# hitfeelee/rtm3d

Measured on AMD Instinct MI355X. Metric: images_per_sec, higher is better.
Workload: dtype fp16

## Files before the change

### rtm3d_amd/csrc/lbfgsb_wave_pub.h

```cpp
#pragma once
#include "lbfgsb.h"
#include "lbfgsb_wave.h"

#if defined(__HIPCC__)
#pragma clang fp contract(off)

namespace lbw_pub {

struct LbWaveMem {
    double ws[LB_N * LB_M], wy[LB_N * LB_M];
    double sy[LB_M * LB_M], ss[LB_M * LB_M], wt[LB_M * LB_M];
    double wn[LB_M2 * LB_M2], wn1d[LB_M2];
    double x[LB_N], z[LB_N], r[LB_N], d[LB_N], t[LB_N], g[LB_N], wv[LB_M2];
    double terms[64], fterms[16], bc[2];
    double uv[16];
#ifdef LBW_PROF
    long long prof[24];
#endif
};
#define VSY_(i, j) w->sy[((j)-1) * LB_M + (i)-1]
#define VSS_(i, j) w->ss[((j)-1) * LB_M + (i)-1]
#define VWT_(i, j) w->wt[((j)-1) * LB_M + (i)-1]
#define VWN_(i, j) w->wn[((j)-1) * LB_M2 + (i)-1]
#define VWN1_(i, j) (*((i) == (j) ? &w->wn1d[(i)-1] : &w->wn[((j)-1) * LB_M2 + (i)-1]))

struct LbWaveK { double k00, k02, k11, k12; };

__device__ static inline int lbw_opaque(int v) {
    asm volatile("" : "+v"(v));
    return v;
}

__device__ static inline int lbw_tri_col(int e) {
    int j = (int)((__fsqrt_rn(8.0f * (float)e + 1.0f) - 1.0f) * 0.5f);
    if ((j + 1) * (j + 2) / 2 <= e) ++j;
    if (j * (j + 1) / 2 > e) --j;
    return j;
}

__device__ static inline double lbw_bcast(double v, int src) {
    int lo = __double2loint(v), hi = __double2hiint(v);
    lo = __builtin_amdgcn_readlane(lo, src);
    hi = __builtin_amdgcn_readlane(hi, src);
    return __hiloint2double(hi, lo);
}

__device__ static inline double lbw_uni(double v) {
    int lo = __double2loint(v), hi = __double2hiint(v);
    lo = __builtin_amdgcn_readfirstlane(lo);
    hi = __builtin_amdgcn_readfirstlane(hi);
    return __hiloint2double(hi, lo);
}

__device__ static inline double lbw_fg(LbWaveMem* w, const LbWaveK& K, int lane) {
    const int c = lane >> 3, i = lane & 7;
    double c0, c1, c2;
    lb_corner(c, &c0, &c1, &c2);
    const double x0 = w->x[0], x1 = w->x[1], x2 = w->x[2], x3 = w->x[3], x4 = w->x[4], x5 = w->x[5], x6 = w->x[6], x7 = w->x[7];
    const double xc = c0 * x2 * x1 + c2 * x4 * x0 + x5;
    const double yc = c1 * x3 + x6;
    const double zc = (-c0) * x2 * x0 + c2 * x4 * x1 + x7;
    const double u = w->uv[2 * c], v = w->uv[2 * c + 1];
    if (i == 0) {
        const double ex = xc * K.k00 / (zc + 1e-4) + K.k02 - u;
        const double ey = yc * K.k11 / (zc + 1e-4) + K.k12 - v;
        w->fterms[2 * c] = ex * ex;
        w->fterms[2 * c + 1] = ey * ey;
    }
    const double dex = (xc * K.k00 / (zc + 1e-6) + K.k02 - u) * 2;
    const double dey = (yc * K.k11 / (zc + 1e-6) + K.k12 - v) * 2;
    double dx, dy, dz;
    switch (i) {
        case 0: dx = c2 * x4; dy = 0; dz = (-c0) * x2; break;
        case 1: dx = c0 * x2; dy = 0; dz = c2 * x4; break;
        case 2: dx = c0 * x1; dy = 0; dz = (-c0) * x0; break;
        case 3: dx = 0; dy = c1; dz = 0; break;
        case 4: dx = c2 * x0; dy = 0; dz = c2 * x1; break;
        case 5: dx = 1; dy = 0; dz = 0; break;
        case 6: dx = 0; dy = 1; dz = 0; break;
        default: dx = 0; dy = 0; dz = 1; break;
    }
    const double den = zc * zc + 1e-6;
    const double gx = K.k00 * (dx * zc - dz * xc) / den;
    const double gy = K.k11 * (dy * zc - dz * yc) / den;
    w->terms[lane] = dex * gx + dey * gy;
    WSYNC();
    if (lane < 8) {
        double s = 0.0;
        for (int k = 0; k < 8; ++k) s += w->terms[k * 8 + lane];
        w->g[lane] = s;
    }
    double f = 0.0;
    for (int k = 0; k < 16; ++k) f += w->fterms[k];
    WSYNC();
    return f;
}

__device__ static inline double lbw_dot8(const double* a, const double* b) {
    double s = 0.0;
    for (int i = 0; i < LB_N; ++i) s += a[i] * b[i];
    return s;
}

template <bool TWO>
__device__ static inline int lbw_potrf_lanes(double* a, int lda, double* b, int ldb, int n, int lane) {
    const int e = lane < (LB_M * (LB_M + 1)) / 2 ? lane : (LB_M * (LB_M + 1)) / 2 - 1;
    const int c = lbw_tri_col(e), r = e - c * (c + 1) / 2;
    const bool act = lane < (LB_M * (LB_M + 1)) / 2 && c < n;
    constexpr bool two = TWO;
    double va = act ? a[c * lda + r] : 0.0, vb = (act && two) ? b[c * ldb + r] : 0.0;
    double da = 0.0, db = 0.0;
    const int src_r = (r * (r + 1) / 2) << 2, src_c = (c * (c + 1) / 2) << 2;
    auto gather = [&](double v, int byte_idx) -> double {
        const int lo = __builtin_amdgcn_ds_bpermute(byte_idx, __double2loint(v));
        const int hi = __builtin_amdgcn_ds_bpermute(byte_idx, __double2hiint(v));
        return __hiloint2double(hi, lo);
    };
    int fail_a = LB_M, fail_b = LB_M;
#pragma unroll
    for (int k = 0; k < LB_M; ++k) {
        if (k < n) {
            const int dk = k * (k + 1) / 2 + k;
            const double pa = va - da, pb = vb - db;
            const double ajj_a = lbw_bcast(pa, dk), ajj_b = two ? lbw_bcast(pb, dk) : 1.0;
            if (!(ajj_a > 0.0) && fail_a == LB_M) fail_a = k;
            if (!(ajj_b > 0.0) && fail_b == LB_M) fail_b = k;
            const double ra = lb_rsqrt(ajj_a), rb = two ? lb_rsqrt(ajj_b) : 0.0;
            const double ua = pa * ra, ub = pb * rb;
            if (act && r == k) { va = c == k ? ra : ua; vb = c == k ? rb : ub; }
            const double ukr_a = gather(ua, src_r + (k << 2)), ukc_a = gather(ua, src_c + (k << 2));
            double ukr_b = 0.0, ukc_b = 0.0;
            if (two) { ukr_b = gather(ub, src_r + (k << 2)); ukc_b = gather(ub, src_c + (k << 2)); }
            if (act && r > k) { da += ukr_a * ukc_a; if (two) db += ukr_b * ukc_b; }
        }
    }
    if (fail_a != LB_M || fail_b != LB_M) return fail_a <= fail_b ? 1 : 2;
    if (act) { a[c * lda + r] = va; if (two) b[c * ldb + r] = vb; }
    WSYNC();
    return 0;
}

__device__ static inline int lbw_trsv_ut(const double* a, int lda, int n, double* b, double* bc, int lane) {
    (void)bc;
    const bool act = lane < n;
    const int col = (act ? lane : 0) * lda;
    double cv[LB_M2];
#pragma unroll
    for (int k = 0; k < LB_M2; ++k) cv[k] = a[col + (k < n ? k : 0)];
    const double dg = a[col + (act ? lane : 0)];
    double bj = act ? b[lane] : 0.0;
    if (__any(act && dg == 0.0)) return 1;
    double dot = 0.0;
#pragma unroll
    for (int k = 0; k < LB_M2; ++k) {
        if (k < n) {
            const double mine = (bj - dot) * dg;
            const double bk = lbw_bcast(mine, k);
            if (lane == k) bj = mine;
            if (lane > k && act) dot += cv[k] * bk;
        }
    }
    if (act) b[lane] = bj;
    WSYNC();
    return 0;
}
__device__ static inline int lbw_trsv_un(const double* a, int lda, int n, double* b, double* bc, int lane) {
    (void)bc;
    const bool act = lane < n;
    const int row = act ? lane : 0;
    constexpr int H = LB_M2 / 2;
    double rh[H], rl[H];
#pragma unroll
    for (int j = 0; j < H; ++j) rh[j] = a[((H + j) < n ? (H + j) : 0) * lda + row];
    const double dg = a[row * lda + row];
    double bk = act ? b[lane] : 0.0;
    if (__any(act && dg == 0.0)) return 1;
#pragma unroll
    for (int j = LB_M2 - 1; j >= 0; --j) {
        if (j == LB_M2 - 6) {
            asm volatile("" ::: "memory");
#pragma unroll
            for (int q = 0; q < H; ++q) rl[q] = a[(q < n ? q : 0) * lda + row];
            asm volatile("" ::: "memory");
        }
        if (j < n) {
            const double mine = bk * dg;
            const double tmp = -lbw_bcast(mine, j);
            if (lane == j) bk = mine;
            if (lane < j) bk += tmp * (j >= H ? rh[j - H] : rl[j]);
        }
    }
    if (act) b[lane] = bk;
    WSYNC();
    return 0;
}

template <bool FULL>
__device__ static inline int lbw_rhs_solve_t(const double* u, double* b, int n) {
    double bv[LB_M], acc[LB_M];
    int bad = 0;
#pragma unroll
    for (int j = 0; j < LB_M; ++j) {
        bv[j] = b[(FULL || j < n) ? j : 0];
        acc[j] = 0.0;
        if ((FULL || j < n) && u[j * LB_M2 + j] == 0.0) bad = 1;
    }
    if (bad) return 1;
#pragma unroll
    for (int J = 0; J < LB_M; ++J) {
        if (FULL || J < n) {
            asm volatile("" ::: "memory");
            double ur[LB_M];
#pragma unroll
            for (int Jp = J; Jp < LB_M; ++Jp) ur[Jp] = u[((FULL || Jp < n) ? Jp : J) * LB_M2 + J];
            const double xJ = (bv[J] - acc[J]) * ur[J];
            bv[J] = xJ;
#pragma unroll
            for (int Jp = J + 1; Jp < LB_M; ++Jp)
                if (FULL || Jp < n) acc[Jp] += ur[Jp] * xJ;
        }
    }
#pragma unroll
    for (int j = 0; j < LB_M; ++j) if (FULL || j < n) b[j] = bv[j];
    return 0;
}
__device__ static inline int lbw_rhs_solve(const double* u, double* b, int n) {
    return n == LB_M ? lbw_rhs_solve_t<true>(u, b, n) : lbw_rhs_solve_t<false>(u, b, n);
}

__device__ static inline int lbw_formk(LbWaveMem* w, int iupdat, double theta, int col, int head, int lane) {
    lane = lbw_opaque(lane);
    const int m = LB_M, n = LB_N;
    PTB(f0_);
    if (iupdat > m) {
        double v[6]; int dr[6], dc[6]; bool ok[6];
#pragma unroll
        for (int r = 0; r < 2; ++r) {
            const int e = lane + 64 * r;
            const bool in = e < (m - 1) * (m - 1);
            const int ee = in ? e : 0;
            const int c = ee / (m - 1) + 1, q = ee % (m - 1) + 1;
            const int qs = q >= c ? q : c;
            ok[3 * r + 0] = in && q >= c; v[3 * r + 0] = VWN1_(qs + 1, c + 1);         dr[3 * r + 0] = qs;     dc[3 * r + 0] = c;
            ok[3 * r + 1] = in && q >= c; v[3 * r + 1] = VWN1_(m + qs + 1, m + c + 1); dr[3 * r + 1] = m + qs; dc[3 * r + 1] = m + c;
            ok[3 * r + 2] = in;           v[3 * r + 2] = VWN1_(m + q + 1, c + 1);      dr[3 * r + 2] = m + q;  dc[3 * r + 2] = c;
        }
        WSYNC();
#pragma unroll
        for (int q = 0; q < 6; ++q) if (ok[q]) VWN1_(dr[q], dc[q]) = v[q];
        WSYNC();
    }
    PTE(f0_, 8); PTB(f1_);
    {
        int ipntr = head + col - 1;
        if (ipntr > m) ipntr -= m;
        const int jy = lane + 1;
        if (jy <= col) {
            const int jpntr = (head + jy - 2) % m + 1;
            double temp1 = 0.0;
            for (int k = 1; k <= n; ++k) temp1 += VWY_(k, ipntr) * VWY_(k, jpntr);
            VWN1_(col, jy) = temp1;
            VWN1_(m + col, m + jy) = 0.0;
            VWN1_(m + col, jy) = 0.0;
        }
        WSYNC();
        const int i = lane + 1;
        if (i <= col) {
            const int ip = (head + i - 2) % m + 1;
            double temp3 = 0.0;
            for (int k = 1; k <= n; ++k) temp3 += VWS_(k, ip) * VWY_(k, ipntr);
            VWN1_(m + i, col) = temp3;
        }
        WSYNC();
    }
    PTE(f1_, 9); PTB(f2_);
    const float rcol = 1.0f / (float)col;
    for (int e = lane; e < col * col; e += 64) {
        const int q = (int)(((float)e + 0.5f) * rcol);
        const int iy = q + 1, jy = e - q * col + 1;
        const int is = col + iy, is1 = m + iy, js = col + jy, js1 = m + jy;
        if (jy <= iy) {
            double v = VWN1_(iy, jy) / theta;
            if (jy == iy) v = v + VSY_(iy, iy);
            VWN_(jy, iy) = v;
            VWN_(js, is) = VWN1_(is1, js1) * theta;
        }
        VWN_(jy, is) = (jy < iy) ? -VWN1_(is1, jy) : VWN1_(is1, jy);
    }
    WSYNC();
    PTE(f2_, 10); PTB(f3_);
    {
        const int r2 = lbw_potrf_lanes<true>(w->wn, LB_M2, w->wt, LB_M, col, lane);
        if (r2 != 0) return r2 == 2 ? -3 : -1;
    }
    PTE(f3_, 11); PTB(f4_);
    const int col2 = 2 * col;
    {
        int bad = 0;
        if (lane < col) bad = lbw_rhs_solve(w->wn, &VWN_(1, col + 1 + lane), col);
        if (__any(bad)) return -1;
        WSYNC();
    }
    PTE(f4_, 12); PTB(f5_);
    {
        const int j = lbw_tri_col(lane);
        const int i = lane - j * (j + 1) / 2;
        if (j < col) {
            const int is = col + 1 + i, js = col + 1 + j;
            double pa[LB_M], pb[LB_M];
#pragma unroll
            for (int k = 1; k <= LB_M; ++k) { const int kk = k <= col ? k : 1; pa[k - 1] = VWN_(kk, is); pb[k - 1] = VWN_(kk, js); }
            double dot = 0.0;
#pragma unroll
            for (int k = 1; k <= LB_M; ++k) if (k <= col) dot += pa[k - 1] * pb[k - 1];
            VWN_(is, js) = VWN_(is, js) + dot;
        }
        WSYNC();
    }
    PTE(f5_, 13); PTB(f6_);
    if (lbw_potrf_lanes<false>(&VWN_(col + 1, col + 1), LB_M2, nullptr, 0, col, lane) != 0) return -2;
    PTE(f6_, 14);
    (void)col2;
    return 0;
}

__device__ static inline int lbw_subsm(LbWaveMem* w, double theta, int col, int head, int lane) {
    lane = lbw_opaque(lane);
    const int m = LB_M, n = LB_N;
    const int col2 = 2 * col;
    if (lane < col2) {
        const int i = (lane < col ? lane : lane - col) + 1;
        const int pointr = (head + i - 2) % m + 1;
        double tmp = 0.0;
        if (lane < col) { for (int j = 1; j <= n; ++j) tmp += VWY_(j, pointr) * w->r[j - 1]; w->wv[lane] = tmp; }
        else { for (int j = 1; j <= n; ++j) tmp += VWS_(j, pointr) * w->r[j - 1]; w->wv[lane] = theta * tmp; }
    }
    WSYNC();
    PTB(s0_);
    if (lbw_trsv_ut(w->wn, LB_M2, col2, w->wv, w->bc, lane) != 0) return 1;
    PTE(s0_, 16);
    if (lane < col) w->wv[lane] = -w->wv[lane];
    WSYNC();
    PTB(s1_);
    if (lbw_trsv_un(w->wn, LB_M2, col2, w->wv, w->bc, lane) != 0) return 1;
    PTE(s1_, 17);
    if (lane < n) {
        double di = w->r[lane];
        int pointr = head;
        const double rt = 1.0 / theta;
#pragma unroll
        for (int h = 0; h < 2; ++h) {
            double ay[LB_M / 2], as[LB_M / 2], vy[LB_M / 2], vs[LB_M / 2];
#pragma unroll
            for (int q = 0; q < LB_M / 2; ++q) {
                const int jy = h * (LB_M / 2) + q + 1;
                const int jj = jy <= col ? jy : 1;
                const int pp = (head + jj - 2) % m + 1;
                ay[q] = VWY_(lane + 1, pp); as[q] = VWS_(lane + 1, pp);
                vy[q] = w->wv[jj - 1]; vs[q] = w->wv[col + jj - 1];
            }
#pragma unroll
            for (int q = 0; q < LB_M / 2; ++q)
                if (h * (LB_M / 2) + q + 1 <= col) di = di + ay[q] * vy[q] * rt + as[q] * vs[q];
        }
        (void)pointr;
        di = rt * di;
        w->r[lane] = di;
        w->z[lane] = w->z[lane] + di;
    }
    WSYNC();
    return 0;
}

__device__ static inline void lbw_matupd(LbWaveMem* w, int* itail, int iupdat, int* col, int* head, double* theta,
                                         double rr, double dr, double stp, double dtd, int lane) {
    lane = lbw_opaque(lane);
    const int m = LB_M, n = LB_N;
    {
        const bool grow = iupdat <= m;
        const int col0 = *col, head0 = *head, itail0 = *itail;
        *col = grow ? iupdat : col0;
        *itail = grow ? (head0 + iupdat - 2) % m + 1 : itail0 % m + 1;
        *head = grow ? head0 : head0 % m + 1;
    }
    if (lane < n) { VWS_(lane + 1, *itail) = w->d[lane]; VWY_(lane + 1, *itail) = w->r[lane]; }
    *theta = rr / dr;
    if (iupdat > m) {
        double vs[2], vy[2]; int dst[2]; bool oks[2], oky[2];
        const int cm = *col - 1;
#pragma unroll
        for (int r = 0; r < 2; ++r) {
            const int e = lane + 64 * r;
            const bool in0 = e < (m - 1) * (m - 1);
            const int ee = in0 ? e : 0;
            const int j = ee / (m - 1) + 1, q = ee % (m - 1) + 1;
            const bool in = in0 && j <= cm && q <= cm;
            oks[r] = in && q <= j; oky[r] = in && q >= j;
            vs[r] = VSS_(q + 1, j + 1); vy[r] = VSY_(q + 1, j + 1);
            dst[r] = (j - 1) * LB_M + (q - 1);
        }
        WSYNC();
#pragma unroll
        for (int r = 0; r < 2; ++r) { if (oks[r]) w->ss[dst[r]] = vs[r]; if (oky[r]) w->sy[dst[r]] = vy[r]; }
    }
    WSYNC();
    const int j = lane + 1;
    if (j <= *col - 1) {
        const int pointr = (*head + j - 2) % m + 1;
        VSY_(*col, j) = lbw_dot8(w->d, &VWY_(1, pointr));
        VSS_(j, *col) = lbw_dot8(&VWS_(1, pointr), w->d);
    }
    if (lane == 0) {
        VSS_(*col, *col) = (stp == 1.0) ? dtd : stp * stp * dtd;
        VSY_(*col, *col) = dr;
    }
    WSYNC();
}

__device__ static inline int lbw_formt(LbWaveMem* w, int col, double theta, int lane) {
    lane = lbw_opaque(lane);
    if (lane < col) w->wv[lane] = 1.0 / VSY_(lane + 1, lane + 1);
    WSYNC();
    const int j0 = lbw_tri_col(lane);
    const int i = lane - j0 * (j0 + 1) / 2 + 1, j = j0 + 1;
    if (j <= col) {
        if (i == 1) VWT_(1, j) = theta * VSS_(1, j);
        else {
            double ddum = 0.0;
#pragma unroll
            for (int h = 0; h < 1; ++h) {
                double pa[9], pb[9], pr[9];
#pragma unroll
                for (int q = 0; q < 9; ++q) {
                    const int k = h * 9 + q + 1;
                    const int kk = k <= i - 1 ? k : 1;
                    pa[q] = VSY_(i, kk); pb[q] = VSY_(j, kk); pr[q] = w->wv[kk - 1];
                }
#pragma unroll
                for (int q = 0; q < 9; ++q) if (h * 9 + q + 1 <= i - 1) ddum = ddum + pa[q] * pb[q] * pr[q];
            }
            VWT_(i, j) = ddum + theta * VSS_(i, j);
        }
    }
    WSYNC();
    return 0;
}

__device__ static inline int lbw_minimize(LbWaveMem* w, const LbWaveK& K, double* f_out, int* nit_out, int lane,
                                          int maxiter, int maxfun) {
    const int n = LB_N, maxls = 20;
    const double epsmch = 2.220446049250313e-16, factr = 1e7, pgtol = 1e-5;
    const double ftol = 1e-3, gtol = 0.9, xtol = 0.1, big = 1e10;
    const double tol = factr * epsmch;
    int col = 0, head = 1, itail = 0, iupdat = 0, updatd = 0, iter = 0, nfgv = 0, info;
    double theta = 1.0, f, fold = 0.0, gd = 0.0, gdold = 0.0, stp = 0.0, dnorm = 0.0, dtd = 0.0, sbgnrm;
    LbSearch S;

#ifdef LBW_PROF
    if (lane < 24) w->prof[lane] = 0;
    WSYNC();
    const long long tstart_ = __builtin_readcyclecounter();
#endif
    f = lbw_uni(lbw_fg(w, K, lane)); nfgv = 1;
    {
        bool finite = lb_isfinite(f);
        for (int i = 0; i < n; ++i) finite = finite && lb_isfinite(w->g[i]);
        if (!finite) { *f_out = f; *nit_out = 0; return LB_STATUS_NONFINITE; }
    }
    sbgnrm = 0.0;
    for (int i = 0; i < n; ++i) sbgnrm = fmax(sbgnrm, fabs(w->g[i]));
    if (sbgnrm <= pgtol) { *f_out = f; *nit_out = 0; return 0; }

    for (;;) {
        if (col == 0) {
            if (lane < n) w->z[lane] = w->x[lane] + 1.0 * (-w->g[lane]);
            WSYNC();
        } else {
            if (lane < n) { w->z[lane] = w->x[lane]; w->r[lane] = -w->g[lane]; }
            WSYNC();
            info = 0;
            PTB(tk_);
            if (updatd) info = lbw_formk(w, iupdat, theta, col, head, lane);
            PTE(tk_, 0); PTB(ts_);
            if (info == 0) info = lbw_subsm(w, theta, col, head, lane);
            PTE(ts_, 1);
            if (info != 0) {
                col = 0; head = 1; theta = 1.0; iupdat = 0; updatd = 0;
                WSYNC();
                continue;
            }
        }
        if (lane < n) { w->d[lane] = w->z[lane] - w->x[lane]; w->t[lane] = w->x[lane]; w->r[lane] = w->g[lane]; }
        WSYNC();
        dtd = lbw_dot8(w->d, w->d);
        dnorm = sqrt(dtd);
        const double stpmx = big;
        stp = (iter == 0) ? fmin(1.0 / dnorm, stpmx) : 1.0;
        fold = f;
        int ifun = 0, iback = 0, ls_fail = 0, start = 1;
        info = 0;
        PTB(tl_);
        for (;;) {
            gd = lbw_dot8(w->g, w->d);
            if (ifun == 0) {
                gdold = gd;
                if (gd >= 0.0) { info = -4; break; }
            }
            const int task = lb_dcsrch(f, gd, &stp, ftol, gtol, xtol, 0.0, stpmx, start, &S);
            start = 0;
            if (task == LS_ERROR) { info = -4; break; }
            if (task == LS_CONV || task == LS_WARN) break;
            ifun += 1; nfgv += 1; iback = ifun - 1;
            WSYNC();
            if (lane < n) w->x[lane] = (stp == 1.0) ? w->z[lane] : stp * w->d[lane] + w->t[lane];
            WSYNC();
            if (iback >= maxls) { ls_fail = 1; break; }
            f = lbw_uni(lbw_fg(w, K, lane));
        }
        PTE(tl_, 2);
        if (info != 0 || ls_fail) {
            WSYNC();
            if (lane < n) { w->x[lane] = w->t[lane]; w->g[lane] = w->r[lane]; }
            WSYNC();
            f = fold;
            if (col == 0) { *f_out = f; *nit_out = iter; return 2; }
            col = 0; head = 1; theta = 1.0; iupdat = 0; updatd = 0;
            continue;
        }
        iter += 1;
        sbgnrm = 0.0;
        for (int i = 0; i < n; ++i) sbgnrm = fmax(sbgnrm, fabs(w->g[i]));
        if (iter >= maxiter || nfgv > maxfun) { *f_out = f; *nit_out = iter; return 1; }
        if (sbgnrm <= pgtol) break;
        const double ddum0 = lb_max3(fabs(fold), fabs(f), 1.0);
        if ((fold - f) <= tol * ddum0) break;
        WSYNC();
        if (lane < n) w->r[lane] = w->g[lane] - w->r[lane];
        WSYNC();
        const double rr = lbw_dot8(w->r, w->r);
        double dr, ddum;
        if (stp == 1.0) { dr = gd - gdold; ddum = -gdold; }
        else {
            dr = (gd - gdold) * stp;
            WSYNC();
            if (lane < n) w->d[lane] = stp * w->d[lane];
            WSYNC();
            ddum = -gdold * stp;
        }
        if (dr <= epsmch * ddum) { updatd = 0; continue; }
        updatd = 1; iupdat += 1;
        PTB(tm_);
        lbw_matupd(w, &itail, iupdat, &col, &head, &theta, rr, dr, stp, dtd, lane);
        theta = lbw_uni(theta);
        PTE(tm_, 3); PTB(tt_);
        if (lbw_formt(w, col, theta, lane) != 0) { col = 0; head = 1; theta = 1.0; iupdat = 0; updatd = 0; }
        PTE(tt_, 4);
    }
    *f_out = f; *nit_out = iter;
#ifdef LBW_PROF
    WSYNC();
    if (lane == 0) w->prof[7] = __builtin_readcyclecounter() - tstart_;
    WSYNC();
    if (lane < 8) w->x[lane] = (double)w->prof[(LBW_PROF - 1) * 8 + lane];
    WSYNC();
#endif
    return 0;
}

}
#endif
```

Baseline: 2560.

## Specialize wave Cholesky and triangular solves for full history, keep solve vector in registers

Adds FULL template specializations of the per-lane Cholesky and the two triangular solves, chosen at runtime when the history is full, so the per-step bound checks disappear. It drops lane masks on accumulations, pairs the two reciprocal square roots into one interleaved Newton-refined routine, and keeps the solve vector in a register between the forward and backward solves, removing an LDS round trip and a barrier. The middle-matrix assembly loop now loads both of its unrolled iterations into registers before a sync and writes afterwards. Dropping the masks relies on inactive lanes producing harmless values, and the new rsqrt refinement can round differently from lb_rsqrt.

```diff
diff --git a/rtm3d_amd/csrc/lbfgsb_wave_pub.h b/rtm3d_amd/csrc/lbfgsb_wave_pub.h
--- a/rtm3d_amd/csrc/lbfgsb_wave_pub.h
+++ b/rtm3d_amd/csrc/lbfgsb_wave_pub.h
@@ -102,11 +102,20 @@
     return s;
 }
 
-template <bool TWO>
-__device__ static inline int lbw_potrf_lanes(double* a, int lda, double* b, int ldb, int n, int lane) {
+__device__ static inline void lbw_rsqrt2(double xa, double xb, double* ra, double* rb) {
+    double ya = __builtin_amdgcn_rsq(xa), yb = __builtin_amdgcn_rsq(xb);
+    const double ha = 0.5 * xa, hb = 0.5 * xb;
+    double ea = fma(-(ha * ya), ya, 0.5), eb = fma(-(hb * yb), yb, 0.5);
+    ya = fma(ya, ea, ya); yb = fma(yb, eb, yb);
+    ea = fma(-(ha * ya), ya, 0.5); eb = fma(-(hb * yb), yb, 0.5);
+    *ra = fma(ya, ea, ya); *rb = fma(yb, eb, yb);
+}
+
+template <bool TWO, bool FULL>
+__device__ static inline int lbw_potrf_lanes_t(double* a, int lda, double* b, int ldb, int n, int lane) {
     const int e = lane < (LB_M * (LB_M + 1)) / 2 ? lane : (LB_M * (LB_M + 1)) / 2 - 1;
     const int c = lbw_tri_col(e), r = e - c * (c + 1) / 2;
-    const bool act = lane < (LB_M * (LB_M + 1)) / 2 && c < n;
+    const bool act = lane < (LB_M * (LB_M + 1)) / 2 && (FULL || c < n);
     constexpr bool two = TWO;
     double va = act ? a[c * lda + r] : 0.0, vb = (act && two) ? b[c * ldb + r] : 0.0;
     double da = 0.0, db = 0.0;
@@ -119,19 +128,20 @@
     int fail_a = LB_M, fail_b = LB_M;
 #pragma unroll
     for (int k = 0; k < LB_M; ++k) {
-        if (k < n) {
+        if (FULL || k < n) {
             const int dk = k * (k + 1) / 2 + k;
             const double pa = va - da, pb = vb - db;
             const double ajj_a = lbw_bcast(pa, dk), ajj_b = two ? lbw_bcast(pb, dk) : 1.0;
             if (!(ajj_a > 0.0) && fail_a == LB_M) fail_a = k;
             if (!(ajj_b > 0.0) && fail_b == LB_M) fail_b = k;
-            const double ra = lb_rsqrt(ajj_a), rb = two ? lb_rsqrt(ajj_b) : 0.0;
+            double ra, rb = 0.0;
+            if (two) lbw_rsqrt2(ajj_a, ajj_b, &ra, &rb); else ra = lb_rsqrt(ajj_a);
             const double ua = pa * ra, ub = pb * rb;
             if (act && r == k) { va = c == k ? ra : ua; vb = c == k ? rb : ub; }
             const double ukr_a = gather(ua, src_r + (k << 2)), ukc_a = gather(ua, src_c + (k << 2));
             double ukr_b = 0.0, ukc_b = 0.0;
             if (two) { ukr_b = gather(ub, src_r + (k << 2)); ukc_b = gather(ub, src_c + (k << 2)); }
-            if (act && r > k) { da += ukr_a * ukc_a; if (two) db += ukr_b * ukc_b; }
+            da += ukr_a * ukc_a; if (two) db += ukr_b * ukc_b;
         }
     }
     if (fail_a != LB_M || fail_b != LB_M) return fail_a <= fail_b ? 1 : 2;
@@ -140,50 +150,54 @@
     return 0;
 }
 
-__device__ static inline int lbw_trsv_ut(const double* a, int lda, int n, double* b, double* bc, int lane) {
-    (void)bc;
+template <bool TWO>
+__device__ static inline int lbw_potrf_lanes(double* a, int lda, double* b, int ldb, int n, int lane) {
+    return n == LB_M ? lbw_potrf_lanes_t<TWO, true>(a, lda, b, ldb, n, lane) : lbw_potrf_lanes_t<TWO, false>(a, lda, b, ldb, n, lane);
+}
+
+template <bool FULL>
+__device__ static inline int lbw_trsv_ut_t(const double* a, int lda, int n, double& bj, int lane) {
     const bool act = lane < n;
     const int col = (act ? lane : 0) * lda;
     double cv[LB_M2];
 #pragma unroll
-    for (int k = 0; k < LB_M2; ++k) cv[k] = a[col + (k < n ? k : 0)];
+    for (int k = 0; k < LB_M2; ++k) cv[k] = a[col + ((FULL || k < n) ? k : 0)];
     const double dg = a[col + (act ? lane : 0)];
-    double bj = act ? b[lane] : 0.0;
     if (__any(act && dg == 0.0)) return 1;
     double dot = 0.0;
 #pragma unroll
     for (int k = 0; k < LB_M2; ++k) {
-        if (k < n) {
+        if (FULL || k < n) {
             const double mine = (bj - dot) * dg;
             const double bk = lbw_bcast(mine, k);
             if (lane == k) bj = mine;
-            if (lane > k && act) dot += cv[k] * bk;
-        }
-    }
-    if (act) b[lane] = bj;
-    WSYNC();
-    return 0;
-}
-__device__ static inline int lbw_trsv_un(const double* a, int lda, int n, double* b, double* bc, int lane) {
-    (void)bc;
+            dot += cv[k] * bk;
+        }
+    }
+    return 0;
+}
+__device__ static inline int lbw_trsv_ut(const double* a, int lda, int n, double& bj, int lane) {
+    return n == LB_M2 ? lbw_trsv_ut_t<true>(a, lda, n, bj, lane) : lbw_trsv_ut_t<false>(a, lda, n, bj, lane);
+}
+template <bool FULL>
+__device__ static inline int lbw_trsv_un_t(const double* a, int lda, int n, double bk, double* b, int lane) {
     const bool act = lane < n;
     const int row = act ? lane : 0;
     constexpr int H = LB_M2 / 2;
     double rh[H], rl[H];
 #pragma unroll
-    for (int j = 0; j < H; ++j) rh[j] = a[((H + j) < n ? (H + j) : 0) * lda + row];
+    for (int j = 0; j < H; ++j) rh[j] = a[((FULL || (H + j) < n) ? (H + j) : 0) * lda + row];
     const double dg = a[row * lda + row];
-    double bk = act ? b[lane] : 0.0;
     if (__any(act && dg == 0.0)) return 1;
 #pragma unroll
     for (int j = LB_M2 - 1; j >= 0; --j) {
         if (j == LB_M2 - 6) {
             asm volatile("" ::: "memory");
 #pragma unroll
-            for (int q = 0; q < H; ++q) rl[q] = a[(q < n ? q : 0) * lda + row];
+            for (int q = 0; q < H; ++q) rl[q] = a[((FULL || q < n) ? q : 0) * lda + row];
             asm volatile("" ::: "memory");
         }
-        if (j < n) {
+        if (FULL || j < n) {
             const double mine = bk * dg;
             const double tmp = -lbw_bcast(mine, j);
             if (lane == j) bk = mine;
@@ -193,6 +207,10 @@
     if (act) b[lane] = bk;
     WSYNC();
     return 0;
+}
+
+__device__ static inline int lbw_trsv_un(const double* a, int lda, int n, double bk, double* b, int lane) {
+    return n == LB_M2 ? lbw_trsv_un_t<true>(a, lda, n, bk, b, lane) : lbw_trsv_un_t<false>(a, lda, n, bk, b, lane);
 }
 
 template <bool FULL>
@@ -275,17 +293,34 @@
     }
     PTE(f1_, 9); PTB(f2_);
     const float rcol = 1.0f / (float)col;
-    for (int e = lane; e < col * col; e += 64) {
-        const int q = (int)(((float)e + 0.5f) * rcol);
-        const int iy = q + 1, jy = e - q * col + 1;
-        const int is = col + iy, is1 = m + iy, js = col + jy, js1 = m + jy;
-        if (jy <= iy) {
-            double v = VWN1_(iy, jy) / theta;
-            if (jy == iy) v = v + VSY_(iy, iy);
-            VWN_(jy, iy) = v;
-            VWN_(js, is) = VWN1_(is1, js1) * theta;
-        }
-        VWN_(jy, is) = (jy < iy) ? -VWN1_(is1, jy) : VWN1_(is1, jy);
+    {
+        double v11[2], v22[2], v12[2]; int iyr[2], jyr[2]; bool in[2];
+#pragma unroll
+        for (int rr = 0; rr < 2; ++rr) {
+            const int e0 = lane + 64 * rr;
+            in[rr] = e0 < col * col;
+            const int e = in[rr] ? e0 : 0;
+            const int q = (int)(((float)e + 0.5f) * rcol);
+            const int iy = q + 1, jy = e - q * col + 1;
+            const int is1 = m + iy;
+            iyr[rr] = iy; jyr[rr] = jy;
+            const int jl = jy <= iy ? jy : iy;
+            v11[rr] = VWN1_(iy, jl); v22[rr] = VWN1_(is1, m + jl); v12[rr] = VWN1_(is1, jy);
+            if (jy == iy) v11[rr] = v11[rr] / theta + VSY_(iy, iy); else v11[rr] = v11[rr] / theta;
+        }
+        WSYNC();
+#pragma unroll
+        for (int rr = 0; rr < 2; ++rr) {
+            const int iy = iyr[rr], jy = jyr[rr];
+            const int is = col + iy, js = col + jy;
+            if (in[rr]) {
+                if (jy <= iy) {
+                    VWN_(jy, iy) = v11[rr];
+                    VWN_(js, is) = v22[rr] * theta;
+                }
+                VWN_(jy, is) = (jy < iy) ? -v12[rr] : v12[rr];
+            }
+        }
     }
     WSYNC();
     PTE(f2_, 10); PTB(f3_);
@@ -337,12 +372,12 @@
     }
     WSYNC();
     PTB(s0_);
-    if (lbw_trsv_ut(w->wn, LB_M2, col2, w->wv, w->bc, lane) != 0) return 1;
+    double wvj = lane < col2 ? w->wv[lane] : 0.0;
+    if (lbw_trsv_ut(w->wn, LB_M2, col2, wvj, lane) != 0) return 1;
     PTE(s0_, 16);
-    if (lane < col) w->wv[lane] = -w->wv[lane];
-    WSYNC();
+    if (lane < col) wvj = -wvj;
     PTB(s1_);
-    if (lbw_trsv_un(w->wn, LB_M2, col2, w->wv, w->bc, lane) != 0) return 1;
+    if (lbw_trsv_un(w->wn, LB_M2, col2, wvj, w->wv, lane) != 0) return 1;
     PTE(s1_, 17);
     if (lane < n) {
         double di = w->r[lane];
```

Result: no change. 2564, median of 6 (+0.2%).
